# qradiolink/qradiolink

Measured on AMD Instinct MI355X. Metric: IQ MSamples/sec through RX demod chain, higher is better.
Workload: dtype f32

## Files before the change

include/qrl_hip.h:

```cpp
#ifndef QRL_HIP_H
#define QRL_HIP_H
#include <stddef.h>
#include <stdint.h>

#ifdef __cplusplus
extern "C" {
#endif

typedef enum {
    QRL_OK = 0,
    QRL_ERR_ARG = -1,
    QRL_ERR_NO_DEVICE = -2,
    QRL_ERR_HIP = -3,
    QRL_ERR_NOMEM = -4,
    QRL_ERR_TOO_BIG = -5,
    QRL_ERR_STATE = -6
} qrl_status;

enum {
    QRL_MODEM_BPSK2K = 0, QRL_MODEM_QPSK20K = 1, QRL_MODEM_QPSKVIDEO = 2, QRL_MODEM_4FSK2K = 3, QRL_MODEM_4FSK10KFM = 4, QRL_MODEM_4FSK2KFM = 5, QRL_MODEM_4FSK1KFM = 6, QRL_MODEM_QPSK2K = 7,
    QRL_MODEM_NBFM2500 = 8, QRL_MODEM_NBFM5000 = 9, QRL_MODEM_WBFM = 10, QRL_MODEM_USB2500 = 11, QRL_MODEM_LSB2500 = 12, QRL_MODEM_CW600USB = 13 , QRL_MODEM_AM5000 = 14,
    QRL_MODEM_2FSK2KFM = 15, QRL_MODEM_2FSK1KFM = 16, QRL_MODEM_2FSK2K = 17, QRL_MODEM_2FSK1K = 18,
    QRL_MODEM_2FSK10KFM = 19, QRL_MODEM_GMSK2K = 20, QRL_MODEM_GMSK1K = 21, QRL_MODEM_GMSK10K = 22,
    QRL_MODEM_BPSK1K = 24, QRL_MODEM_BPSK8 = 25 , QRL_MODEM_QPSK250K = 26, QRL_MODEM_4FSK100K = 27, QRL_MODEM_M17 = 40, QRL_MODEM_DMR = 41
// ... 8 lines not shown
const char* qrl_last_error(void);
const char* qrl_version(void);

typedef struct {
    int modem_type;
    int use_mode_defaults;
    int sps, samp_rate, carrier_freq, filter_width, fm;
    int device_samp_rate;
    double carrier_offset_hz;
    int batch;
    size_t max_chunk;
    void* hip_stream;
    int enable_side_outputs;
    int time_domain_samp_rate;
    double time_domain_filter_width;
} qrl_demod_config;

typedef struct {
    float* filtered;      size_t filtered_cap;
    float* constellation; size_t constellation_cap;
    uint8_t* bits_a;      size_t bits_cap;
    uint8_t* bits_b;
    uint32_t* counts;
    float* audio;         size_t audio_cap;
} qrl_demod_out;

int qrl_demod_create(qrl_ctx* ctx, const qrl_demod_config* cfg, qrl_demod** out);
void qrl_demod_destroy(qrl_demod* d);
int qrl_demod_reset(qrl_demod* d);
int qrl_demod_set_carrier_offset(qrl_demod* d, double carrier_offset_hz);
int qrl_demod_set_carrier_offsets(qrl_demod* d, const double* hz);
#define QRL_DMO_RECORD_BYTES 40
int qrl_demod_set_dmo_output(qrl_demod* d, uint8_t* frames, size_t cap_frames, uint32_t* counts);
enum { QRL_OPT_OVERLAP = 1, QRL_OPT_UNFUSED_DEC2 = 2, QRL_OPT_FLL_SLIM = 3 , QRL_OPT_GROUPED = 4, QRL_OPT_INPUT_RESIDENT = 5 };
int qrl_demod_set_option(qrl_demod* d, int option, int value);
int qrl_demod_out_caps(const qrl_demod* d, size_t n, size_t* filtered_cap, size_t* constellation_cap, size_t* bits_cap);
int qrl_demod_audio_cap(const qrl_demod* d, size_t n, size_t* audio_cap);
int qrl_demod_set_squelch(qrl_demod* d, double db);
int qrl_demod_time_domain_cap(const qrl_demod* d, size_t n, size_t* cap);
int qrl_demod_set_time_domain_output(qrl_demod* d, float* samples, size_t cap, uint32_t* counts);
int qrl_demod_set_ctcss(qrl_demod* d, float tone_hz);
int qrl_demod_set_agc(qrl_demod* d, float attack, float decay);
int qrl_demod_set_filter_width(qrl_demod* d, int filter_width);
int qrl_demod_set_gain(qrl_demod* d, float value);

int qrl_demod_process(qrl_demod* d, const float* iq, size_t stride, size_t n, const qrl_demod_out* out);
int qrl_demod_process_sc16(qrl_demod* d, const int16_t* iq, size_t stride, size_t n, const qrl_demod_out* out);
int qrl_demod_set_sc16_scale(qrl_demod* d, float scale);
int qrl_demod_sync(qrl_demod* d);
void* qrl_demod_stream(qrl_demod* d);
int qrl_demod_internal_streams(qrl_demod* d, void* out[3]);
int qrl_demod_stream_wait(qrl_demod* d, void* hip_stream);

int qrl_demod_profile(qrl_demod* d, int enable);
int qrl_demod_profile_read(qrl_demod* d, double* kernel_ms, uint64_t* launches, const char** kernel_name);

int qrl_demod_process_host(qrl_demod* d, const float* iq_host, size_t stride, size_t n,
                           uint8_t* bits_a_host, uint8_t* bits_b_host, size_t bits_cap, uint32_t* counts_host);
int qrl_demod_process_sc16_host(qrl_demod* d, const int16_t* iq_host, size_t stride, size_t n,
                                uint8_t* bits_a_host, uint8_t* bits_b_host, size_t bits_cap, uint32_t* counts_host);

typedef struct qrl_mod qrl_mod;
typedef struct {
    int modem_type;
    int use_mode_defaults;
    int sps, samp_rate, carrier_freq, filter_width, fm;
    int batch;
// ... 178 lines not shown
```

qradiolink_amd/__init__.py:

```python
import ctypes as C
import os

import numpy as np

_HERE = os.path.dirname(os.path.abspath(__file__))
LIB_PATH = os.environ.get("QRL_LIB_PATH") or os.path.join(_HERE, "libqrl_hip.so")

MODEM_2FSK2KFM, MODEM_2FSK1KFM, MODEM_2FSK2K, MODEM_2FSK1K, MODEM_2FSK10KFM = 15, 16, 17, 18, 19
MODEM_GMSK2K, MODEM_GMSK1K, MODEM_GMSK10K = 20, 21, 22
MODEM_QPSK250K = 26
MODEM_QPSK20K, MODEM_QPSKVIDEO, MODEM_QPSK2K = 1, 2, 7
MODEM_BPSK2K, MODEM_BPSK1K = 0, 24
MODEM_4FSK2K, MODEM_4FSK10KFM, MODEM_4FSK2KFM, MODEM_4FSK1KFM, MODEM_4FSK100K = 3, 4, 5, 6, 27
MODEM_BPSK8 = 25
MODEM_NBFM2500, MODEM_NBFM5000, MODEM_WBFM, MODEM_AM5000 = 8, 9, 10, 14
MODEM_USB2500, MODEM_LSB2500, MODEM_CW600USB = 11, 12, 13
MODEM_M17 = 40
MODEM_DMR = 41
OPT_OVERLAP, OPT_UNFUSED_DEC2, OPT_FLL_SLIM, OPT_GROUPED, OPT_INPUT_RESIDENT = 1, 2, 3, 4, 5
CHAN_OPT_LEGACY_PFB, CHAN_OPT_LEGACY_TAIL, CHAN_OPT_SERIAL_TAIL = 1, 2, 3
WIN_HAMMING, WIN_HANN, WIN_BLACKMAN, WIN_RECTANGULAR, WIN_BLACKMAN_HARRIS = 0, 1, 2, 3, 5


class QrlError(RuntimeError):
    pass


class _Config(C.Structure):
    _fields_ = [("modem_type", C.c_int), ("use_mode_defaults", C.c_int), ("sps", C.c_int), ("samp_rate", C.c_int),
                ("carrier_freq", C.c_int), ("filter_width", C.c_int), ("fm", C.c_int), ("device_samp_rate", C.c_int),
                ("carrier_offset_hz", C.c_double), ("batch", C.c_int), ("max_chunk", C.c_size_t),
                ("hip_stream", C.c_void_p), ("enable_side_outputs", C.c_int), ("time_domain_samp_rate", C.c_int), ("time_domain_filter_width", C.c_double)]


class _ModConfig(C.Structure):
    _fields_ = [("modem_type", C.c_int), ("use_mode_defaults", C.c_int), ("sps", C.c_int), ("samp_rate", C.c_int),
                ("carrier_freq", C.c_int), ("filter_width", C.c_int), ("fm", C.c_int), ("batch", C.c_int),
                ("max_bytes", C.c_size_t), ("hip_stream", C.c_void_p), ("bb_gain", C.c_float),
                ("device_samp_rate", C.c_int), ("carrier_offset_hz", C.c_double)]


class _ChanConfig(C.Structure):
    _fields_ = [("num_channels", C.c_int), ("channel_first", C.c_int), ("channel_count", C.c_int), ("batch", C.c_int),
                ("max_chunk", C.c_size_t), ("hip_stream", C.c_void_p), ("form", C.c_int), ("channel_separation", C.c_int),
                ("decimation", C.c_int), ("filter_width", C.c_int)]


class _SynthConfig(C.Structure):
    _fields_ = [("num_channels", C.c_int), ("filter_width", C.c_int), ("batch", C.c_int), ("max_samples", C.c_size_t),
                ("hip_stream", C.c_void_p), ("bb_gain", C.c_float), ("single_carrier", C.c_int)]


# ... 1029 lines not shown
```

qradiolink_amd/csrc/demod.hpp:

```cpp
#pragma once
#include "host_common.hpp"
#include "firdes.hpp"
#include <utility>

namespace qrl {

inline std::vector<float> decim_layout(const std::vector<float>& h, int D, int Jpad)
{
    std::vector<float> t((size_t)D * Jpad, 0.0f);
    for (size_t k = 0; k < h.size(); ++k) t[(k % D) * Jpad + k / D] = h[k];
    return t;
}
inline std::vector<float> resamp_layout(const std::vector<float>& h, int I, int Jp)
{
    std::vector<float> t((size_t)I * Jp, 0.0f);
    for (size_t k = 0; k < h.size(); ++k) t[(k % I) * Jp + k / I] = h[k];
    return t;
}
inline std::vector<float2> to_f2(const std::vector<std::complex<float>>& v)
{
    std::vector<float2> r(v.size());
    for (size_t i = 0; i < v.size(); ++i) r[i] = make_float2(v[i].real(), v[i].imag());
    return r;
}
// ... 63 lines not shown
    DevBuf<float> rs, filt, mf; int Jp = 0, nf = 0;
    DevBuf<float2> ra, rb, rc, rd, sym; uint32_t mask = 0, sym_mask = 0;
    DevBuf<DsssState> st; DevBuf<DsssTailState> tail;
    float a1 = 0, b1 = 0, a2 = 0, b2 = 0;
    uint64_t n5 = 0, nsy = 0;
    int build(qrl_demod& d, size_t max2);
    int init_state(qrl_demod& d);
    int stages(qrl_demod& d, uint64_t n2_0, uint64_t n2_1, const qrl_demod_out* out, uint32_t* counts);
};

}

using namespace qrl;

struct qrl_demod {
    qrl_ctx* ctx = nullptr;
    qrl_demod_config cfg{};
    hipStream_t stream = nullptr;
    bool own_stream = false;
    hipStream_t tail = nullptr;
    hipStream_t fecs = nullptr;
    hipEvent_t ev_q[2] = {nullptr, nullptr}, ev_fec[2] = {nullptr, nullptr}; bool q_valid[2] = {false, false};
    bool grouped = false, grouped_capable = false, fec_deferred = false; FecParams fec_pending{}; int fec_pending_slot = 0;
    DevBuf<uint64_t> qp_snap;
    hipEvent_t ev_ff = nullptr, ev_tail = nullptr;
    hipStream_t pre = nullptr; hipEvent_t ev_pre = nullptr, ev_fe[2] = {nullptr, nullptr}; bool fe_valid[2] = {false, false}; bool pre_pending = false;
    bool input_resident = false;
    hipEvent_t ev_user[4] = {nullptr, nullptr, nullptr, nullptr};
    bool tail_pending = false;
    bool qpsk_fll = false, fsk4_disc = false;
    bool m17 = false;
    DevBuf<float2> s2g, disc4_taps; DevBuf<float> sym4_taps; int disc4_nt = 0, sym4_nt = 0;
    bool fll_slim = false;
    bool d2f_capable = false, d2f = false; DevBuf<float> d2f_taps;
    bool overlap = false, overlap_capable = false; hipEvent_t ev_tail2[2] = {nullptr, nullptr}; bool tail2_valid[2] = {false, false}; uint64_t call_no = 0;
    enum Family { F_2FSK, F_GMSK, F_QPSK, F_DMR, F_4FSK, F_BPSK, F_DSSS, F_ANALOG } fam = F_2FSK;
    int branches = 2;

    int fe_decim = 1, interp = 1, decim = 1, target = 0, sps_eff = 0;
    bool fm = false;

    DecimStage fe;
    DecimStage first;
    DecimStage scope; DevBuf<float2> s_scope; uint32_t scope_mask = 0; uint64_t n_scope = 0; int scope_D = 10;
    float2* scope_out = nullptr; size_t scope_cap = 0; uint32_t* scope_counts = nullptr;
    DevBuf<float> rs_taps; int rs_Jp = 0;
    DevBuf<float> filt_taps; int filt_nt = 0;
    DevBuf<float> symf_taps; int symf_nt = 0;
    DevBuf<float2> disc_up, disc_lo; int disc_nt = 0;
    DevBuf<float> ff_tf, ff_ts; DevBuf<float2> ff_up, ff_lo;
    DevBuf<float2> fll_lo, fll_up; float fll_alpha = 0, fll_beta = 0, fll_maxf = 0;
    DevBuf<float> atan_tab, mmse_tab;
    float demod_gain = 0;
    float ss_alpha = 0, ss_beta = 0, ss_maxp = 0, ss_minp = 0;

    Rotator rot;

    DevBuf<float2> hist_a, hist_b; uint32_t hist_len = 0; bool hist_flip = false;
    DevBuf<float2> s1, s2, s2l, s2f; DevBuf<float> s2d, s3; DevBuf<uint8_t> soft;
    uint32_t s1_mask = 0, s2_mask = 0, soft_mask = 0;
    DevBuf<FllState> fll_st; DevBuf<SymSyncState> ss_st; DevBuf<FecState> fec_st;
    DevBuf<DmoState> dmo_st; DevBuf<uint32_t> dmo_golay; uint8_t* dmo_out = nullptr; uint32_t dmo_cap = 0; uint32_t* dmo_counts = nullptr;
    DevBuf<QpskState> qp_st; DevBuf<float> tanh_tab;
    float c1_alpha = 0, c1_beta = 0, c2_alpha = 0, c2_beta = 0; float2 qp_rot{};
    DevBuf<uint32_t> counts_scratch;
    AnalogChain an;
// ... 49 lines not shown
```

qradiolink_amd/csrc/engine.cpp:

```cpp
#include "demod.hpp"
#include <cmath>
#include <cstdlib>
#include <memory>
#include <new>

#ifndef QRL_FEC_GATE_US
#define QRL_FEC_GATE_US 30u
#endif
#ifndef QRL_DEV_SKIP
#define QRL_DEV_SKIP 0
#endif

int qrl_demod::flush_fec(bool behind_front_end)
{
    if (!fec_deferred) return QRL_OK;
    fec_deferred = false;
    HIPCHK(hipStreamWaitEvent(fecs, ev_q[fec_pending_slot], 0));
    if (behind_front_end) {
        HIPCHK(hipStreamWaitEvent(fecs, ev_ff, 0));
        launch_fec_gate(QRL_FEC_GATE_US, fecs);
    }
    launch_fec(fec_pending, cfg.batch, fecs);
    HIPCHK(hipEventRecord(ev_fec[fec_pending_slot], fecs));
    return QRL_OK;
// ... 359 lines not shown
    {
        HistParams h{};
        h.in = in; h.in_stride = stride; h.n0 = n_in0; h.n = (uint32_t)n;
        h.hist_old = hist_old; h.hist_new = hist_new; h.hist_len = hist_len;
        h.rot_enable = 1; rot.fill(h);
        h.in_fmt = fmt; h.in_scale = sc16_scale;
        if (pre) { HIPCHK(hipEventRecord(ev_fe[slot], stream)); fe_valid[slot] = true; }
        if (use_pre) {
            if (fe_valid[slot ^ 1]) HIPCHK(hipStreamWaitEvent(pre, ev_fe[slot ^ 1], 0));
            launch_hist_save(h, B, pre);
            HIPCHK(hipEventRecord(ev_pre, pre));
            pre_pending = true;
        } else launch_hist_save(h, B, stream);
        hist_flip = !hist_flip;
    }
    if (overlap) {
        HIPCHK(hipEventRecord(ev_ff, stream));
        HIPCHK(hipStreamWaitEvent(tail, ev_ff, 0));
        HIPCHK(hipMemsetAsync(counts, 0, (size_t)B * 4 * sizeof(uint32_t), tail));
    }
    const uint32_t c2 = (uint32_t)(n2_1 - n2_0);
    if (fam == F_DSSS || fam == F_ANALOG) {
        if (int rr = fam == F_DSSS ? ds.stages(*this, n2_0, n2_1, out, counts) : an.stages(*this, n2_0, n2_1, out, counts)) return rr;
        HIPCHK(hipGetLastError());
        if (take_launch_error()) return QRL_ERR_HIP;
        n_in = n_in1; n1 = n1_1; n2 = n2_1; ++call_no;
        return QRL_OK;
    }
    RingC filt_in = r2;
    if (fam == F_2FSK || fam == F_BPSK || (fam == F_QPSK && qpsk_fll)) {
        FllParams f{};
        f.in = r2; f.out = r2l; f.q0 = n2_0; f.count = c2; f.st = fll_st.p;
        f.lower = fll_lo.p; f.upper = fll_up.p; f.nt = fam == F_2FSK ? 16 : 32; f.alpha = fll_alpha; f.beta = fll_beta; f.max_freq = fll_maxf;
        f.slim = fll_slim ? 1 : 0;
        if (!(QRL_DEV_SKIP & 1)) launch_fll(f, B, cs);
        filt_in = r2l;
    }
    const bool fused_2fsk = fam == F_2FSK && !fm && filt_nt <= 41 && disc_nt <= 41 && symf_nt <= 25;
    if (fam == F_DMR) {
        RingC dem_in = r2;
        if (m17) {
            FirCcfParams f{};
            f.in = r2; f.out = r2f; f.q0 = n2_0; f.count = c2; f.taps = filt_taps.p; f.nt = filt_nt;
            f.port = fport.p; f.port_cap = fport.cap; f.counts = counts;
            launch_fir_ccf(f, B, cs);
            dem_in = r2f;
        }
        QuadDemodParams q{}; q.in = dem_in; q.out = r2d; q.q0 = n2_0; q.count = c2; q.gain = demod_gain; q.atan_tab = atan_tab.p;
        launch_quad_demod(q, B, cs);
        if (!overlap && tail_pending) { HIPCHK(hipStreamWaitEvent(stream, ev_tail, 0)); tail_pending = false; }
        FirFffParams f{}; f.in = r2d; f.out = r3; f.q0 = n2_0; f.count = c2; f.taps = symf_taps.p; f.nt = symf_nt;
        launch_fir_fff(f, B, cs);
        if (!overlap) { HIPCHK(hipEventRecord(ev_ff, stream)); HIPCHK(hipStreamWaitEvent(tail, ev_ff, 0)); }
    } else if (fused_2fsk) {
        if (!overlap && tail_pending) { HIPCHK(hipStreamWaitEvent(stream, ev_tail, 0)); tail_pending = false; }
        Fsk2FfParams f{};
        f.in = filt_in; f.out = r3; f.q0 = n2_0; f.count = c2;
        f.tf = ff_tf.p; f.nf = fsk2_ff_padded(filt_nt); f.up = ff_up.p; f.lo = ff_lo.p; f.nb = fsk2_ff_padded(disc_nt);
        f.ts = ff_ts.p; f.ns = fsk2_ff_padded(symf_nt);
        f.port = fport.p; f.port_cap = fport.cap; f.counts = counts;
        if (!(QRL_DEV_SKIP & 2)) launch_2fsk_ff(f, B, cs);
        if (!overlap) { HIPCHK(hipEventRecord(ev_ff, stream)); HIPCHK(hipStreamWaitEvent(tail, ev_ff, 0)); }
    } else {
        if (!d2f) {
            FirCcfParams f{};
            f.in = filt_in; f.out = r2f; f.q0 = n2_0; f.count = c2; f.taps = filt_taps.p; f.nt = filt_nt;
            f.port = fport.p; f.port_cap = fport.cap; f.counts = counts;
// ... 228 lines not shown
    HIPCHK(hipEventRecord(d->ev_user[3], d->pre ? d->pre : d->stream));
    for (auto e : d->ev_user) HIPCHK(hipStreamWaitEvent(user, e, 0));
    return QRL_OK;
}
int qrl_demod_set_dmo_output(qrl_demod* d, uint8_t* frames, size_t cap_frames, uint32_t* counts)
{
    if (!d) return QRL_ERR_ARG;
    if (d->fam != qrl_demod::F_DMR || d->m17) return qrl_set_error(QRL_ERR_ARG, "the DMO slicer sits behind port 3 of gr_demod_dmr: QRL_MODEM_DMR only");
    if (!frames) { if (int rs = d->sync_all()) return rs; d->dmo_out = nullptr; return QRL_OK; }
    if (!counts || cap_frames < 1 || cap_frames > 0xFFFFFFFFu) return QRL_ERR_ARG;
    int r;
    if (!d->dmo_st.p) {
        if (int rs = d->sync_all()) return rs;
        if ((r = d->dmo_st.alloc(d->cfg.batch)) || (r = d->dmo_golay.upload(golay1987_table()))) return r;
        if ((r = d->init_dmo_state())) return r;
    }
    d->dmo_out = frames; d->dmo_cap = (uint32_t)cap_frames; d->dmo_counts = counts;
    return QRL_OK;
}
int qrl_demod_set_option(qrl_demod* d, int option, int value)
{
    if (!d) return QRL_ERR_ARG;
    switch (option) {
    case QRL_OPT_OVERLAP:
        if (value != 0 && !d->overlap_capable) return qrl_set_error(QRL_ERR_ARG, "overlapped mode exists for the 2FSK family only");
        if (int rs = d->sync_all()) return rs;
        d->overlap = value != 0;
        d->tail2_valid[0] = d->tail2_valid[1] = false;
        return QRL_OK;
    case QRL_OPT_FLL_SLIM:
        if (int rs = d->sync_all()) return rs;
        d->fll_slim = value != 0;
        return QRL_OK;
    case QRL_OPT_GROUPED:
        if (value != 0 && !d->grouped_capable) return qrl_set_error(QRL_ERR_ARG, "the grouped order exists for the gr_demod_qpsk chain only");
        if (int rs = d->sync_all()) return rs;
        d->grouped = value != 0;
        return QRL_OK;
    case QRL_OPT_INPUT_RESIDENT: {
        if (int rs = d->sync_all()) return rs;
        if (value != 0 && d->pre) {
            DecimStage& st = d->fe.used ? d->fe : d->first;
            if (st.edge_len && !st.edge_b.p) if (int r = st.edge_b.alloc((size_t)d->cfg.batch * st.edge_len)) return qrl_set_error(r, "edge scratch");
        }
        d->input_resident = value != 0;
        return QRL_OK;
    }
    case QRL_OPT_UNFUSED_DEC2:
        if (!d->d2f_capable) return qrl_set_error(QRL_ERR_ARG, "this chain has no fused 1:2 decimator + shaping filter");
        if (d->n_in != 0) return qrl_set_error(QRL_ERR_STATE, "QRL_OPT_UNFUSED_DEC2 can only be set before the first sample (the two forms carry different state)");
        d->d2f = value == 0;
        return QRL_OK;
    default:
        return qrl_set_error(QRL_ERR_ARG, "unknown option");
    }
}
int qrl_demod_out_caps(const qrl_demod* d, size_t n, size_t* fcap, size_t* ccap, size_t* bcap)
{
    if (!d) return QRL_ERR_ARG;
    const CallCounts cc = d->call_counts(n);
    const size_t ns = cc.nsym;
    if (fcap) *fcap = cc.n2;
    if (ccap) *ccap = ns;
    if (bcap) *bcap = d->fam == qrl_demod::F_DMR ? 2 * ns + 8 : d->fam == qrl_demod::F_QPSK || d->fam == qrl_demod::F_4FSK ? (ns / 80 + 2) * 80 : (ns / 2 / 80 + 2) * 80;
    return QRL_OK;
}
// ... 141 lines not shown
```

qradiolink_amd/csrc/engine.hpp:

```cpp
#pragma once
#include <hip/hip_runtime.h>
#include <stdint.h>
#include <vector>
#include "zero_runs.hpp"
#include "decim_plan.hpp"

namespace qrl {

hipError_t dyn_lds_limit(const void* kernel, int bytes);
bool take_launch_error();

int create_role_stream(hipStream_t* s, int priority, const char* role);

struct RingC { float2* p; uint32_t mask; };
struct RingF { float* p; uint32_t mask; };
struct RingB { uint8_t* p; uint32_t mask; };

template <class Pp>
__device__ __forceinline__ void rot_select(Pp& c, const Pp& p, uint32_t b)
{
    c = p; c.rot_acc = p.rot_acc_s[b]; c.rot_inc = p.rot_inc_s[b]; c.rot_lo = p.rot_lo + (size_t)b * 512;
}
#define ROT_VIEW(T, PS, P, SRC, B) T P##_ps_; if constexpr (PS) rot_select(P##_ps_, SRC, (uint32_t)(B)); const T& P = (PS) ? P##_ps_ : SRC
std::vector<float2> rot_fine_table(uint64_t inc);
// ... 73 lines not shown
    RingC in_ring;
    RingC out;
    uint64_t q0; uint32_t q_count;
    const float* taps;
    int I, D, Jp;
    int rot_enable; uint64_t rot_acc; uint64_t rot_inc; uint64_t rot_nbase; const float2* rot_lo;
    float2* port; size_t port_cap; uint32_t* port_counts;
    const uint64_t* rot_acc_s; const uint64_t* rot_inc_s;
};
void launch_resamp(const ResampParams& p, int batch, hipStream_t s);

struct FirCcfParams { RingC in; RingC out; uint64_t q0; uint32_t count; const float* taps; int nt;
                      float2* port; size_t port_cap; uint32_t* counts; };
struct FirFffParams { RingF in; RingF out; uint64_t q0; uint32_t count; const float* taps; int nt; };
struct QuadDemodParams { RingC in; RingF out; uint64_t q0; uint32_t count; float gain; const float* atan_tab;
                         RingF out2; float gain2;
                         int16_t* s16; size_t s16_cap; float s16_level, s16_scale; uint32_t* s16_counts; };
struct Disc2fskParams { RingC in; RingF out; uint64_t q0; uint32_t count; const float2* up; const float2* lo; int nt; };
struct Disc4fskParams { RingC in; RingC out; uint64_t q0; uint32_t count; const float2* taps; int nt; };
void launch_disc_4fsk(const Disc4fskParams& p, int batch, hipStream_t s);
struct Fsk2FfParams { RingC in; RingF out; uint64_t q0; uint32_t count;
                      const float* tf; int nf; const float2* up; const float2* lo; int nb; const float* ts; int ns;
                      float2* port; size_t port_cap; uint32_t* counts; };
void launch_2fsk_ff(const Fsk2FfParams& p, int batch, hipStream_t s);
int fsk2_ff_padded(int n);
void launch_fir_ccf(const FirCcfParams& p, int batch, hipStream_t s);
void launch_fir_fff(const FirFffParams& p, int batch, hipStream_t s);
void launch_quad_demod(const QuadDemodParams& p, int batch, hipStream_t s);
void launch_disc_2fsk(const Disc2fskParams& p, int batch, hipStream_t s);

struct FllState { float phase, freq; float2 dl[32]; };
struct FllParams { RingC in; RingC out; uint64_t q0; uint32_t count; FllState* st;
                   const float2* lower; const float2* upper; int nt; float alpha, beta, max_freq;
                   int slim; };
void launch_fll(const FllParams& p, int batch, hipStream_t s);

struct SymSyncState { uint64_t ii; uint64_t oo; float mu, avg, inst; float x0, x1, x2, d0, d1, d2; };
struct SymSyncParams {
    RingF in; uint64_t avail;
    RingB soft;
    SymSyncState* st;
    const float* mmse;
    float alpha, beta, maxp, minp;
    int ted; float soft_mul, soft_add;
    int slicer;
    float tail_scale;
    int tail;
    uint8_t* bits; size_t bits_cap;
    float2* port; size_t port_cap; uint32_t* counts;
    int slim;
};
void launch_symsync_ff(const SymSyncParams& p, int batch, hipStream_t s);

struct QpskState {
    uint64_t ii, oo;
    float gain;
    float c1_phase, c1_freq;
    float mu, avg, inst;
    float2 x0, x1, x2, d0, d1, d2;
    float c2_phase, c2_freq;
    float2 dprev;
    float2 hist[16];
};
struct QpskParams {
    RingC in; uint64_t np0, avail;
    RingB soft; QpskState* st;
    const float* mmse; const float* tanh_tab;
// ... 203 lines not shown
```

qradiolink_amd/csrc/kernels_ff.hip:

```cpp
#include "devmath.hpp"
#include "engine.hpp"
#include <cstdlib>

namespace qrl {

__device__ __forceinline__ float2 ringc_at(const RingC& r, int b, int64_t i)
{
    if (i < 0) return make_float2(0.f, 0.f);
    return r.p[(size_t)b * (r.mask + 1u) + ((uint32_t)i & r.mask)];
}
__device__ __forceinline__ float ringf_at(const RingF& r, int b, int64_t i)
{
    if (i < 0) return 0.f;
    return r.p[(size_t)b * (r.mask + 1u) + ((uint32_t)i & r.mask)];
}

__global__ __launch_bounds__(256) void k_fir_ccf(const FirCcfParams P)
{
    const int b = blockIdx.y;
    const uint32_t t = blockIdx.x * 256u + threadIdx.x;
    if (t >= P.count) return;
    if (t == 0 && P.counts) P.counts[b * 4 + 0] = P.count;
    const int64_t n = (int64_t)(P.q0 + t);
    float ar = 0.f, ai = 0.f;
// ... 198 lines not shown
    ItemT cur[4], nxt[4];
#pragma unroll
    for (int s = 0; s < 4; ++s) cur[s] = tile[s * PITCH + w];
    auto quad = [&](int q) {
        --w;
#pragma unroll
        for (int s = 0; s < 4; ++s) nxt[s] = tile[s * PITCH + w];
        const TapT h0 = taps[4 * q], h1 = taps[4 * q + 1], h2 = taps[4 * q + 2], h3 = taps[4 * q + 3];
        fma4(h0, cur[0], cur[1], cur[2], cur[3]);
        fma4(h1, nxt[3], cur[0], cur[1], cur[2]);
        fma4(h2, nxt[2], nxt[3], cur[0], cur[1]);
        fma4(h3, nxt[1], nxt[2], nxt[3], cur[0]);
#pragma unroll
        for (int s = 0; s < 4; ++s) cur[s] = nxt[s];
    };
    if constexpr (NQ > 0) {
#pragma unroll 4
        for (int q = 0; q < NQ; ++q) quad(q);
    } else {
        for (int q = 0; q < nq_rt; ++q) quad(q);
    }
}

template <int NQF, int NQB, int NQS>
__global__ __launch_bounds__(256) void k_2fsk_ff(const Fsk2FfParams P)
{
    __shared__ float2 lt[4 * FF_PL];
    __shared__ float2 ft[4 * FF_PF];
    __shared__ float dt[4 * FF_PD];
    const int b = blockIdx.y, tid = threadIdx.x;
    const int hf = P.nf - 1, hb = P.nb - 1, hs = P.ns - 1;
    const int T = 1024 - hb - hs;
    const int64_t n0t = (int64_t)P.q0 + (int64_t)blockIdx.x * T;
    const int nl = 1024 + hf, nd = T + hs;
    if (tid < 4) { lt[tid * FF_PL] = make_float2(0.f, 0.f); ft[tid * FF_PF] = make_float2(0.f, 0.f); dt[tid * FF_PD] = 0.f; }
    {
        float2 v[5];
#pragma unroll
        for (int it = 0; it < 5; ++it) {
            const int64_t a = n0t - (hf + hb + hs) + tid + 256 * it;
            v[it] = P.in.p[(size_t)b * (P.in.mask + 1u) + ((uint32_t)a & P.in.mask)];
            if (a < 0) v[it] = make_float2(0.f, 0.f);
        }
#pragma unroll
        for (int it = 0; it < 5; ++it) {
            const int i = tid + 256 * it;
            if (i < nl) lt[(i & 3) * FF_PL + (i >> 2) + 1] = v[it];
        }
    }
    __syncthreads();
    {
        float2 a[4] = {{0.f, 0.f}, {0.f, 0.f}, {0.f, 0.f}, {0.f, 0.f}};
        ff_window4<FF_PL, NQF>(lt, tid + (hf >> 2) + 1, (hf >> 2) + 1, P.tf,
                          [&](float h, const float2& x0, const float2& x1, const float2& x2, const float2& x3) {
                              a[0].x = fmaf(h, x0.x, a[0].x); a[0].y = fmaf(h, x0.y, a[0].y);
                              a[1].x = fmaf(h, x1.x, a[1].x); a[1].y = fmaf(h, x1.y, a[1].y);
                              a[2].x = fmaf(h, x2.x, a[2].x); a[2].y = fmaf(h, x2.y, a[2].y);
                              a[3].x = fmaf(h, x3.x, a[3].x); a[3].y = fmaf(h, x3.y, a[3].y);
                          });
#pragma unroll
        for (int r = 0; r < 4; ++r) {
            const bool neg = n0t - (hb + hs) + 4 * tid + r < 0;
            ft[r * FF_PF + tid + 1] = neg ? make_float2(0.f, 0.f) : a[r];
        }
    }
    __syncthreads();
    if (4 * tid < nd) {
        float ar[4] = {0.f, 0.f, 0.f, 0.f}, ai[4] = {0.f, 0.f, 0.f, 0.f}, br[4] = {0.f, 0.f, 0.f, 0.f}, bi[4] = {0.f, 0.f, 0.f, 0.f};
        const int nq = NQB > 0 ? NQB : (hb >> 2) + 1;
        int w = tid + (hb >> 2) + 1;
        float2 cur[4], nxt[4];
#pragma unroll
        for (int s = 0; s < 4; ++s) cur[s] = ft[s * FF_PF + w];
        auto step = [&](const float2 h, const float2& x0, const float2& x1, const float2& x2, const float2& x3) {
            const float2 xs[4] = {x0, x1, x2, x3};
#pragma unroll
            for (int r = 0; r < 4; ++r) {
                ar[r] = fmaf(h.x, xs[r].x, ar[r]); ai[r] = fmaf(h.x, xs[r].y, ai[r]);
                br[r] = fmaf(h.y, xs[r].x, br[r]); bi[r] = fmaf(h.y, xs[r].y, bi[r]);
            }
        };
        auto quad = [&](int q) {
            --w;
#pragma unroll
            for (int s = 0; s < 4; ++s) nxt[s] = ft[s * FF_PF + w];
            step(P.up[4 * q], cur[0], cur[1], cur[2], cur[3]);
            step(P.up[4 * q + 1], nxt[3], cur[0], cur[1], cur[2]);
            step(P.up[4 * q + 2], nxt[2], nxt[3], cur[0], cur[1]);
            step(P.up[4 * q + 3], nxt[1], nxt[2], nxt[3], cur[0]);
#pragma unroll
            for (int s = 0; s < 4; ++s) cur[s] = nxt[s];
        };
        if constexpr (NQB > 0) {
#pragma unroll 4
            for (int q = 0; q < NQB; ++q) quad(q);
        } else {
            for (int q = 0; q < nq; ++q) quad(q);
        }
#pragma unroll
        for (int r = 0; r < 4; ++r) {
            const float ur = ar[r] - bi[r], ui = ai[r] + br[r], lr = ar[r] + bi[r], li = ai[r] - br[r];
            const float mu = sqrtf(ur * ur + ui * ui);
            const float ml = sqrtf(lr * lr + li * li);
            float v = mu / ml;
            if (!(v >= 0.0f)) v = 0.0f;
            if (v > 2.0f) v = 2.0f;
            dt[r * FF_PD + tid + 1] = (n0t - hs + 4 * tid + r < 0) ? 0.f : v + (-1.0f);
        }
    }
    __syncthreads();
    if (4 * tid < T) {
        float a[4] = {0.f, 0.f, 0.f, 0.f};
        ff_window4<FF_PD, NQS>(dt, tid + (hs >> 2) + 1, (hs >> 2) + 1, P.ts,
                          [&](float h, float x0, float x1, float x2, float x3) {
                              a[0] = fmaf(h, x0, a[0]); a[1] = fmaf(h, x1, a[1]); a[2] = fmaf(h, x2, a[2]); a[3] = fmaf(h, x3, a[3]);
                          });
        const uint32_t t0 = blockIdx.x * (uint32_t)T + 4u * tid;
        if (t0 == 0 && P.counts) P.counts[b * 4 + 0] = P.count;
        const int wf = tid + ((hb + hs) >> 2) + 1;
#pragma unroll
        for (int r = 0; r < 4; ++r) {
            const uint32_t t = t0 + r;
            if (t < P.count) {
                const int64_t n = n0t + 4 * tid + r;
                P.out.p[(size_t)b * (P.out.mask + 1u) + ((uint32_t)n & P.out.mask)] = a[r];
                if (P.port && t < P.port_cap) P.port[(size_t)b * P.port_cap + t] = ft[r * FF_PF + wf];
            }
        }
    }
}
int fsk2_ff_padded(int n) { return (n - 1 + 3) / 4 * 4 + 1; }
void launch_2fsk_ff(const Fsk2FfParams& p, int batch, hipStream_t s)
{
    if (!p.count) return;
    const int T = 1024 - (p.nb - 1) - (p.ns - 1);
    const dim3 grid((p.count + T - 1) / T, batch);
    static const bool rt = [] { const char* e = getenv("QRL_FF_RUNTIME_TAPS"); return e && atoi(e) != 0; }();
    const int qf = (p.nf - 1) / 4 + 1, qb = (p.nb - 1) / 4 + 1, qs = (p.ns - 1) / 4 + 1;
    if (!rt && qf == 11 && qb == 11 && qs == 7) hipLaunchKernelGGL((k_2fsk_ff<11, 11, 7>), grid, dim3(256), 0, s, p);
    else hipLaunchKernelGGL((k_2fsk_ff<0, 0, 0>), grid, dim3(256), 0, s, p);
}

}
```

qradiolink_amd/csrc/kernels_loops.hip:

```cpp
#include "devmath.hpp"
#include "engine.hpp"

namespace qrl {


#ifndef QRL_FLL_CH
#define QRL_FLL_CH 32
#endif
#ifndef QRL_FLL_TH
#define QRL_FLL_TH 256
#endif
template <int CTRL> __device__ __forceinline__ float dpp_quad(float v)
{
    return __builtin_bit_cast(float, __builtin_amdgcn_mov_dpp(__builtin_bit_cast(int, v), CTRL, 0xF, 0xF, true));
}

template <int NT, int FLL_TH, int FLL_CH>
__global__ __launch_bounds__(FLL_TH) void k_fll(const FllParams P, int batch)
{
    constexpr int FLL_NS = FLL_TH / 4;
    constexpr int GL = NT / 4;
    __shared__ float2 win[FLL_NS][FLL_CH + 1];
    __shared__ float2 tl[NT], tu[NT];
    __shared__ float2 dump[FLL_TH];
    const int tid = threadIdx.x;
    const int sl = tid >> 2, g = tid & 3;
    const int b0 = blockIdx.x * FLL_NS;
    const int b = b0 + sl;
    const bool active = b < batch;
    for (int k = tid; k < NT; k += FLL_TH) { tl[k] = P.lower[k]; tu[k] = P.upper[k]; }
    float phase = 0.f, freq = 0.f;
    float2 dl[GL];
    if (active) {
        const FllState& s = P.st[b];
        phase = s.phase; freq = s.freq;
#pragma unroll
        for (int t = 0; t < GL; ++t) dl[t] = s.dl[g * GL + t];
    } else {
#pragma unroll
        for (int t = 0; t < GL; ++t) dl[t] = make_float2(0.f, 0.f);
    }
    const int nstreams = min(FLL_NS, batch - b0);
    __syncthreads();
    float2 hu[GL], hl[GL];
#pragma unroll
    for (int t = 0; t < GL; ++t) { hu[t] = tu[g * GL + t]; hl[t] = tl[g * GL + t]; }
    constexpr int NPT = FLL_NS * FLL_CH / FLL_TH;
    float2 pre[NPT];
    auto preload = [&](uint32_t c0) {
#pragma unroll
        for (int i = 0; i < NPT; ++i) {
            const int idx = tid + FLL_TH * i, s = min(idx / FLL_CH, nstreams - 1), k = idx % FLL_CH;
            const int64_t a = (int64_t)(P.q0 + c0 + k) - NT;
            const float2 v = P.in.p[(size_t)(b0 + s) * (P.in.mask + 1u) + ((uint32_t)a & P.in.mask)];
            pre[i] = a >= 0 ? v : make_float2(0.f, 0.f);
        }
    };
    preload(0);
    for (uint32_t c0 = 0; c0 < P.count; c0 += FLL_CH) {
        const int len = min((uint32_t)FLL_CH, P.count - c0);
        __syncthreads();
#pragma unroll
        for (int i = 0; i < NPT; ++i) { const int idx = tid + FLL_TH * i; win[idx / FLL_CH][idx % FLL_CH] = pre[i]; }
        __syncthreads();
        if (c0 + FLL_CH < P.count) preload(c0 + FLL_CH);
        if (active) {
            for (int k = 0; k < len; ++k) {
                const float2 x = win[sl][k];
                const float2 nco = sincos_rad(phase);
                float2 carry;
                carry.x = dpp_quad<0x90>(dl[GL - 1].x);
                carry.y = dpp_quad<0x90>(dl[GL - 1].y);
#pragma unroll
                for (int t = GL - 1; t > 0; --t) dl[t] = dl[t - 1];
                float ur = 0.f, ui = 0.f, lr = 0.f, li = 0.f;
#pragma unroll
                for (int t = GL - 1; t >= 1; --t) {
                    const float2 v = dl[t];
                    ur = fmaf(hu[t].x, v.x, ur); ur = fmaf(-hu[t].y, v.y, ur);
                    ui = fmaf(hu[t].x, v.y, ui); ui = fmaf(hu[t].y, v.x, ui);
                    lr = fmaf(hl[t].x, v.x, lr); lr = fmaf(-hl[t].y, v.y, lr);
                    li = fmaf(hl[t].x, v.y, li); li = fmaf(hl[t].y, v.x, li);
                }
                const float2 y = cmul(x, nco);
                *(g == 0 ? &win[sl][k] : &dump[tid]) = y;
                dl[0] = g == 0 ? y : carry;
                {
                    const float2 v = dl[0];
                    ur = fmaf(hu[0].x, v.x, ur); ur = fmaf(-hu[0].y, v.y, ur);
                    ui = fmaf(hu[0].x, v.y, ui); ui = fmaf(hu[0].y, v.x, ui);
                    lr = fmaf(hl[0].x, v.x, lr); lr = fmaf(-hl[0].y, v.y, lr);
                    li = fmaf(hl[0].x, v.y, li); li = fmaf(hl[0].y, v.x, li);
                }
                ur = ur + dpp_quad<0xB1>(ur); ui = ui + dpp_quad<0xB1>(ui); lr = lr + dpp_quad<0xB1>(lr); li = li + dpp_quad<0xB1>(li);
                ur = ur + dpp_quad<0x4E>(ur); ui = ui + dpp_quad<0x4E>(ui); lr = lr + dpp_quad<0x4E>(lr); li = li + dpp_quad<0x4E>(li);
                const float error = (lr * lr + li * li) - (ur * ur + ui * ui);
                freq = freq + P.beta * error;
                phase = phase + freq + P.alpha * error;
                phase = phase_wrap(phase);
                freq = __builtin_fminf(__builtin_fmaxf(freq, -P.max_freq), P.max_freq);
            }
        }
        __syncthreads();
#pragma unroll
        for (int i = 0; i < NPT; ++i) {
            const int idx = tid + FLL_TH * i, s = idx / FLL_CH, k = idx % FLL_CH;
            if (s < nstreams && k < len) P.out.p[(size_t)(b0 + s) * (P.out.mask + 1u) + ((uint32_t)(P.q0 + c0 + k) & P.out.mask)] = win[s][k];
        }
    }
    if (active) {
        FllState& s = P.st[b];
        if (g == 0) { s.phase = phase; s.freq = freq; }
#pragma unroll
        for (int t = 0; t < GL; ++t) s.dl[g * GL + t] = dl[t];
    }
}

void launch_fll(const FllParams& p, int batch, hipStream_t s)
{
    if (!p.count) return;
    if (p.slim) {
        dim3 grid((batch + 15) / 16), block(64);
        if (p.nt == 16) hipLaunchKernelGGL((k_fll<16, 64, 16>), grid, block, 0, s, p, batch);
        else            hipLaunchKernelGGL((k_fll<32, 64, 16>), grid, block, 0, s, p, batch);
        return;
    }
    constexpr int TH = QRL_FLL_TH;
    dim3 grid((batch + TH / 4 - 1) / (TH / 4)), block(TH);
    if (p.nt == 16) hipLaunchKernelGGL((k_fll<16, TH, QRL_FLL_CH>), grid, block, 0, s, p, batch);
    else            hipLaunchKernelGGL((k_fll<32, TH, QRL_FLL_CH>), grid, block, 0, s, p, batch);
}

template <int NS, int W> struct SsGeo {
    static constexpr int BACK = 16;
    static constexpr int COLS = BACK + W + 8;
    static constexpr int PITCH = COLS + 1;
    static constexpr int OMAX = W == 192 ? 56 : (W + 5) * 2 / 7 + 1;
    static constexpr int OPITCH = OMAX + 1;
    static constexpr size_t lds_bytes() { return (size_t)(2 * NS * PITCH + 4 + 129 * 8 + 2 * NS * OPITCH) * sizeof(float) + 2 * 64 * sizeof(int) + (2 * 64 + 64 + 2) * sizeof(uint64_t); }
};

__device__ __forceinline__ uint64_t wave_min_u64(uint64_t v)
{
#pragma unroll
    for (int off = 32; off > 0; off >>= 1) {
        const uint64_t o = __shfl_xor((unsigned long long)v, off, 64);
        v = o < v ? o : v;
    }
    return v;
}

template <int SS_NS, int SS_W, bool VEC = false, int SS_TH = 256>
__global__ __launch_bounds__(SS_TH) void k_symsync_ff(const SymSyncParams P, int batch)
{
    using G = SsGeo<SS_NS, SS_W>;
    constexpr int SS_BACK = G::BACK, SS_COLS = G::COLS, SS_PITCH = G::PITCH, SS_OMAX = G::OMAX, SS_OPITCH = G::OPITCH;
    extern __shared__ __align__(16) unsigned char ss_smem[];
    float* win = reinterpret_cast<float*>(ss_smem);
    float* mm = win + 2 * SS_NS * SS_PITCH + 4;
    float* osym = mm + 129 * 8;
    int* ocnt = reinterpret_cast<int*>(osym + 2 * SS_NS * SS_OPITCH);
    uint64_t* obase = reinterpret_cast<uint64_t*>(ocnt + 2 * 64);
    uint64_t* oo0 = obase + 2 * 64;
// ... 233 lines not shown
```

Baseline: 535,000.

## Make FLL lanes-per-stream configurable and trim FF kernel tail work

Generalizes the FLL band-edge kernel so each stream can be handled by 1, 2 or 4 lanes, with a new option and compile-time defaults that pick the lane count. Fewer lanes per stream mean fewer cross-lane DPP reductions and more streams per block, at the cost of more serial FMAs per lane. The defaults stay at 4 lanes, so the default path matches the old layout apart from the refactor into a step lambda. Separately, the fused FF kernel now bounds its loads and compute loops by the valid sample count of the last block, which skips loads and filtering past the end of the data.

```diff
diff --git a/include/qrl_hip.h b/include/qrl_hip.h
--- a/include/qrl_hip.h
+++ b/include/qrl_hip.h
@@ -64,7 +64,8 @@
 int qrl_demod_set_carrier_offsets(qrl_demod* d, const double* hz);
 #define QRL_DMO_RECORD_BYTES 40
 int qrl_demod_set_dmo_output(qrl_demod* d, uint8_t* frames, size_t cap_frames, uint32_t* counts);
-enum { QRL_OPT_OVERLAP = 1, QRL_OPT_UNFUSED_DEC2 = 2, QRL_OPT_FLL_SLIM = 3 , QRL_OPT_GROUPED = 4, QRL_OPT_INPUT_RESIDENT = 5 };
+enum { QRL_OPT_OVERLAP = 1, QRL_OPT_UNFUSED_DEC2 = 2, QRL_OPT_FLL_SLIM = 3 , QRL_OPT_GROUPED = 4, QRL_OPT_INPUT_RESIDENT = 5,
+       QRL_OPT_FLL_LANES = 6  };
 int qrl_demod_set_option(qrl_demod* d, int option, int value);
 int qrl_demod_out_caps(const qrl_demod* d, size_t n, size_t* filtered_cap, size_t* constellation_cap, size_t* bits_cap);
 int qrl_demod_audio_cap(const qrl_demod* d, size_t n, size_t* audio_cap);
diff --git a/qradiolink_amd/__init__.py b/qradiolink_amd/__init__.py
--- a/qradiolink_amd/__init__.py
+++ b/qradiolink_amd/__init__.py
@@ -17,7 +17,7 @@
 MODEM_USB2500, MODEM_LSB2500, MODEM_CW600USB = 11, 12, 13
 MODEM_M17 = 40
 MODEM_DMR = 41
-OPT_OVERLAP, OPT_UNFUSED_DEC2, OPT_FLL_SLIM, OPT_GROUPED, OPT_INPUT_RESIDENT = 1, 2, 3, 4, 5
+OPT_OVERLAP, OPT_UNFUSED_DEC2, OPT_FLL_SLIM, OPT_GROUPED, OPT_INPUT_RESIDENT, OPT_FLL_LANES = 1, 2, 3, 4, 5, 6
 CHAN_OPT_LEGACY_PFB, CHAN_OPT_LEGACY_TAIL, CHAN_OPT_SERIAL_TAIL = 1, 2, 3
 WIN_HAMMING, WIN_HANN, WIN_BLACKMAN, WIN_RECTANGULAR, WIN_BLACKMAN_HARRIS = 0, 1, 2, 3, 5
 
diff --git a/qradiolink_amd/csrc/demod.hpp b/qradiolink_amd/csrc/demod.hpp
--- a/qradiolink_amd/csrc/demod.hpp
+++ b/qradiolink_amd/csrc/demod.hpp
@@ -119,6 +119,7 @@
     bool m17 = false;
     DevBuf<float2> s2g, disc4_taps; DevBuf<float> sym4_taps; int disc4_nt = 0, sym4_nt = 0;
     bool fll_slim = false;
+    int fll_lanes = 0;
     bool d2f_capable = false, d2f = false; DevBuf<float> d2f_taps;
     bool overlap = false, overlap_capable = false; hipEvent_t ev_tail2[2] = {nullptr, nullptr}; bool tail2_valid[2] = {false, false}; uint64_t call_no = 0;
     enum Family { F_2FSK, F_GMSK, F_QPSK, F_DMR, F_4FSK, F_BPSK, F_DSSS, F_ANALOG } fam = F_2FSK;
diff --git a/qradiolink_amd/csrc/engine.cpp b/qradiolink_amd/csrc/engine.cpp
--- a/qradiolink_amd/csrc/engine.cpp
+++ b/qradiolink_amd/csrc/engine.cpp
@@ -415,7 +415,7 @@
         FllParams f{};
         f.in = r2; f.out = r2l; f.q0 = n2_0; f.count = c2; f.st = fll_st.p;
         f.lower = fll_lo.p; f.upper = fll_up.p; f.nt = fam == F_2FSK ? 16 : 32; f.alpha = fll_alpha; f.beta = fll_beta; f.max_freq = fll_maxf;
-        f.slim = fll_slim ? 1 : 0;
+        f.slim = fll_slim ? 1 : 0; f.lanes = fll_lanes;
         if (!(QRL_DEV_SKIP & 1)) launch_fll(f, B, cs);
         filt_in = r2l;
     }
@@ -710,6 +710,11 @@
         if (int rs = d->sync_all()) return rs;
         d->fll_slim = value != 0;
         return QRL_OK;
+    case QRL_OPT_FLL_LANES:
+        if (value != 1 && value != 2 && value != 4) return qrl_set_error(QRL_ERR_ARG, "QRL_OPT_FLL_LANES takes 1, 2 or 4");
+        if (int rs = d->sync_all()) return rs;
+        d->fll_lanes = value;
+        return QRL_OK;
     case QRL_OPT_GROUPED:
         if (value != 0 && !d->grouped_capable) return qrl_set_error(QRL_ERR_ARG, "the grouped order exists for the gr_demod_qpsk chain only");
         if (int rs = d->sync_all()) return rs;
diff --git a/qradiolink_amd/csrc/engine.hpp b/qradiolink_amd/csrc/engine.hpp
--- a/qradiolink_amd/csrc/engine.hpp
+++ b/qradiolink_amd/csrc/engine.hpp
@@ -129,7 +129,8 @@
 struct FllState { float phase, freq; float2 dl[32]; };
 struct FllParams { RingC in; RingC out; uint64_t q0; uint32_t count; FllState* st;
                    const float2* lower; const float2* upper; int nt; float alpha, beta, max_freq;
-                   int slim; };
+                   int slim;
+                   int lanes; };
 void launch_fll(const FllParams& p, int batch, hipStream_t s);
 
 struct SymSyncState { uint64_t ii; uint64_t oo; float mu, avg, inst; float x0, x1, x2, d0, d1, d2; };
diff --git a/qradiolink_amd/csrc/kernels_ff.hip b/qradiolink_amd/csrc/kernels_ff.hip
--- a/qradiolink_amd/csrc/kernels_ff.hip
+++ b/qradiolink_amd/csrc/kernels_ff.hip
@@ -254,24 +254,25 @@
     const int hf = P.nf - 1, hb = P.nb - 1, hs = P.ns - 1;
     const int T = 1024 - hb - hs;
     const int64_t n0t = (int64_t)P.q0 + (int64_t)blockIdx.x * T;
-    const int nl = 1024 + hf, nd = T + hs;
+    const int nv = (int)min((uint32_t)T, P.count - blockIdx.x * (uint32_t)T);
+    const int n1 = nv + hb + hs, n2 = nv + hs;
     if (tid < 4) { lt[tid * FF_PL] = make_float2(0.f, 0.f); ft[tid * FF_PF] = make_float2(0.f, 0.f); dt[tid * FF_PD] = 0.f; }
     {
         float2 v[5];
 #pragma unroll
         for (int it = 0; it < 5; ++it) {
             const int64_t a = n0t - (hf + hb + hs) + tid + 256 * it;
-            v[it] = P.in.p[(size_t)b * (P.in.mask + 1u) + ((uint32_t)a & P.in.mask)];
-            if (a < 0) v[it] = make_float2(0.f, 0.f);
+            v[it] = make_float2(0.f, 0.f);
+            if (tid + 256 * it < n1 + hf && a >= 0) v[it] = P.in.p[(size_t)b * (P.in.mask + 1u) + ((uint32_t)a & P.in.mask)];
         }
 #pragma unroll
         for (int it = 0; it < 5; ++it) {
             const int i = tid + 256 * it;
-            if (i < nl) lt[(i & 3) * FF_PL + (i >> 2) + 1] = v[it];
-        }
-    }
-    __syncthreads();
-    {
+            if (i < n1 + hf) lt[(i & 3) * FF_PL + (i >> 2) + 1] = v[it];
+        }
+    }
+    __syncthreads();
+    if (4 * tid < n1) {
         float2 a[4] = {{0.f, 0.f}, {0.f, 0.f}, {0.f, 0.f}, {0.f, 0.f}};
         ff_window4<FF_PL, NQF>(lt, tid + (hf >> 2) + 1, (hf >> 2) + 1, P.tf,
                           [&](float h, const float2& x0, const float2& x1, const float2& x2, const float2& x3) {
@@ -287,7 +288,7 @@
         }
     }
     __syncthreads();
-    if (4 * tid < nd) {
+    if (4 * tid < n2) {
         float ar[4] = {0.f, 0.f, 0.f, 0.f}, ai[4] = {0.f, 0.f, 0.f, 0.f}, br[4] = {0.f, 0.f, 0.f, 0.f}, bi[4] = {0.f, 0.f, 0.f, 0.f};
         const int nq = NQB > 0 ? NQB : (hb >> 2) + 1;
         int w = tid + (hb >> 2) + 1;
@@ -331,7 +332,7 @@
         }
     }
     __syncthreads();
-    if (4 * tid < T) {
+    if (4 * tid < nv) {
         float a[4] = {0.f, 0.f, 0.f, 0.f};
         ff_window4<FF_PD, NQS>(dt, tid + (hs >> 2) + 1, (hs >> 2) + 1, P.ts,
                           [&](float h, float x0, float x1, float x2, float x3) {
diff --git a/qradiolink_amd/csrc/kernels_loops.hip b/qradiolink_amd/csrc/kernels_loops.hip
--- a/qradiolink_amd/csrc/kernels_loops.hip
+++ b/qradiolink_amd/csrc/kernels_loops.hip
@@ -15,36 +15,39 @@
     return __builtin_bit_cast(float, __builtin_amdgcn_mov_dpp(__builtin_bit_cast(int, v), CTRL, 0xF, 0xF, true));
 }
 
-template <int NT, int FLL_TH, int FLL_CH>
+template <int NT, int FLL_TH, int FLL_CH, int LPS = 4>
 __global__ __launch_bounds__(FLL_TH) void k_fll(const FllParams P, int batch)
 {
-    constexpr int FLL_NS = FLL_TH / 4;
+    static_assert(LPS == 1 || LPS == 2 || LPS == 4, "lanes per stream");
+    constexpr int FLL_NS = FLL_TH / LPS;
     constexpr int GL = NT / 4;
+    constexpr int CPL = 4 / LPS;
+    constexpr int ML = CPL * GL;
     __shared__ float2 win[FLL_NS][FLL_CH + 1];
     __shared__ float2 tl[NT], tu[NT];
-    __shared__ float2 dump[FLL_TH];
+    __shared__ float2 dump[LPS == 4 ? FLL_TH : LPS == 2 ? FLL_NS : 1];
     const int tid = threadIdx.x;
-    const int sl = tid >> 2, g = tid & 3;
+    const int sl = tid / LPS, g = tid % LPS;
     const int b0 = blockIdx.x * FLL_NS;
     const int b = b0 + sl;
     const bool active = b < batch;
     for (int k = tid; k < NT; k += FLL_TH) { tl[k] = P.lower[k]; tu[k] = P.upper[k]; }
     float phase = 0.f, freq = 0.f;
-    float2 dl[GL];
+    float2 dl[ML];
     if (active) {
         const FllState& s = P.st[b];
         phase = s.phase; freq = s.freq;
 #pragma unroll
-        for (int t = 0; t < GL; ++t) dl[t] = s.dl[g * GL + t];
+        for (int t = 0; t < ML; ++t) dl[t] = s.dl[g * ML + t];
     } else {
 #pragma unroll
-        for (int t = 0; t < GL; ++t) dl[t] = make_float2(0.f, 0.f);
+        for (int t = 0; t < ML; ++t) dl[t] = make_float2(0.f, 0.f);
     }
     const int nstreams = min(FLL_NS, batch - b0);
     __syncthreads();
-    float2 hu[GL], hl[GL];
-#pragma unroll
-    for (int t = 0; t < GL; ++t) { hu[t] = tu[g * GL + t]; hl[t] = tl[g * GL + t]; }
+    float2 hu[ML], hl[ML];
+#pragma unroll
+    for (int t = 0; t < ML; ++t) { hu[t] = tu[g * ML + t]; hl[t] = tl[g * ML + t]; }
     constexpr int NPT = FLL_NS * FLL_CH / FLL_TH;
     float2 pre[NPT];
     auto preload = [&](uint32_t c0) {
@@ -56,6 +59,57 @@
             pre[i] = a >= 0 ? v : make_float2(0.f, 0.f);
         }
     };
+    auto step = [&](int k) __attribute__((always_inline)) {
+        const float2 x = win[sl][k];
+        const float2 nco = sincos_rad(phase);
+        float2 carry = make_float2(0.f, 0.f);
+        if constexpr (LPS == 4) { carry.x = dpp_quad<0x90>(dl[ML - 1].x); carry.y = dpp_quad<0x90>(dl[ML - 1].y); }
+        if constexpr (LPS == 2) { carry.x = dpp_quad<0xA0>(dl[ML - 1].x); carry.y = dpp_quad<0xA0>(dl[ML - 1].y); }
+#pragma unroll
+        for (int t = ML - 1; t > 0; --t) dl[t] = dl[t - 1];
+        float ur[CPL], ui[CPL], lr[CPL], li[CPL];
+#pragma unroll
+        for (int c = CPL - 1; c >= 0; --c) {
+            ur[c] = 0.f; ui[c] = 0.f; lr[c] = 0.f; li[c] = 0.f;
+#pragma unroll
+            for (int t = c * GL + GL - 1; t >= c * GL + (c == 0 ? 1 : 0); --t) {
+                const float2 v = dl[t];
+                ur[c] = fmaf(hu[t].x, v.x, ur[c]); ur[c] = fmaf(-hu[t].y, v.y, ur[c]);
+                ui[c] = fmaf(hu[t].x, v.y, ui[c]); ui[c] = fmaf(hu[t].y, v.x, ui[c]);
+                lr[c] = fmaf(hl[t].x, v.x, lr[c]); lr[c] = fmaf(-hl[t].y, v.y, lr[c]);
+                li[c] = fmaf(hl[t].x, v.y, li[c]); li[c] = fmaf(hl[t].y, v.x, li[c]);
+            }
+        }
+        const float2 y = cmul(x, nco);
+        if constexpr (LPS == 4) *(g == 0 ? &win[sl][k] : &dump[tid]) = y;
+        if constexpr (LPS == 2) *(g == 0 ? &win[sl][k] : &dump[sl]) = y;
+        if constexpr (LPS == 1) win[sl][k] = y;
+        if constexpr (LPS == 1) dl[0] = y; else dl[0] = g == 0 ? y : carry;
+        {
+            const float2 v = dl[0];
+            ur[0] = fmaf(hu[0].x, v.x, ur[0]); ur[0] = fmaf(-hu[0].y, v.y, ur[0]);
+            ui[0] = fmaf(hu[0].x, v.y, ui[0]); ui[0] = fmaf(hu[0].y, v.x, ui[0]);
+            lr[0] = fmaf(hl[0].x, v.x, lr[0]); lr[0] = fmaf(-hl[0].y, v.y, lr[0]);
+            li[0] = fmaf(hl[0].x, v.y, li[0]); li[0] = fmaf(hl[0].y, v.x, li[0]);
+        }
+        float sur, sui, slr, sli;
+        if constexpr (LPS == 1) {
+            sur = (ur[0] + ur[1]) + (ur[2] + ur[3]); sui = (ui[0] + ui[1]) + (ui[2] + ui[3]);
+            slr = (lr[0] + lr[1]) + (lr[2] + lr[3]); sli = (li[0] + li[1]) + (li[2] + li[3]);
+        } else if constexpr (LPS == 2) {
+            sur = ur[0] + ur[1]; sui = ui[0] + ui[1]; slr = lr[0] + lr[1]; sli = li[0] + li[1];
+            sur = sur + dpp_quad<0xB1>(sur); sui = sui + dpp_quad<0xB1>(sui); slr = slr + dpp_quad<0xB1>(slr); sli = sli + dpp_quad<0xB1>(sli);
+        } else {
+            sur = ur[0]; sui = ui[0]; slr = lr[0]; sli = li[0];
+            sur = sur + dpp_quad<0xB1>(sur); sui = sui + dpp_quad<0xB1>(sui); slr = slr + dpp_quad<0xB1>(slr); sli = sli + dpp_quad<0xB1>(sli);
+            sur = sur + dpp_quad<0x4E>(sur); sui = sui + dpp_quad<0x4E>(sui); slr = slr + dpp_quad<0x4E>(slr); sli = sli + dpp_quad<0x4E>(sli);
+        }
+        const float error = (slr * slr + sli * sli) - (sur * sur + sui * sui);
+        freq = freq + P.beta * error;
+        phase = phase + freq + P.alpha * error;
+        phase = phase_wrap(phase);
+        freq = __builtin_fminf(__builtin_fmaxf(freq, -P.max_freq), P.max_freq);
+    };
     preload(0);
     for (uint32_t c0 = 0; c0 < P.count; c0 += FLL_CH) {
         const int len = min((uint32_t)FLL_CH, P.count - c0);
@@ -65,41 +119,7 @@
         __syncthreads();
         if (c0 + FLL_CH < P.count) preload(c0 + FLL_CH);
         if (active) {
-            for (int k = 0; k < len; ++k) {
-                const float2 x = win[sl][k];
-                const float2 nco = sincos_rad(phase);
-                float2 carry;
-                carry.x = dpp_quad<0x90>(dl[GL - 1].x);
-                carry.y = dpp_quad<0x90>(dl[GL - 1].y);
-#pragma unroll
-                for (int t = GL - 1; t > 0; --t) dl[t] = dl[t - 1];
-                float ur = 0.f, ui = 0.f, lr = 0.f, li = 0.f;
-#pragma unroll
-                for (int t = GL - 1; t >= 1; --t) {
-                    const float2 v = dl[t];
-                    ur = fmaf(hu[t].x, v.x, ur); ur = fmaf(-hu[t].y, v.y, ur);
-                    ui = fmaf(hu[t].x, v.y, ui); ui = fmaf(hu[t].y, v.x, ui);
-                    lr = fmaf(hl[t].x, v.x, lr); lr = fmaf(-hl[t].y, v.y, lr);
-                    li = fmaf(hl[t].x, v.y, li); li = fmaf(hl[t].y, v.x, li);
-                }
-                const float2 y = cmul(x, nco);
-                *(g == 0 ? &win[sl][k] : &dump[tid]) = y;
-                dl[0] = g == 0 ? y : carry;
-                {
-                    const float2 v = dl[0];
-                    ur = fmaf(hu[0].x, v.x, ur); ur = fmaf(-hu[0].y, v.y, ur);
-                    ui = fmaf(hu[0].x, v.y, ui); ui = fmaf(hu[0].y, v.x, ui);
-                    lr = fmaf(hl[0].x, v.x, lr); lr = fmaf(-hl[0].y, v.y, lr);
-                    li = fmaf(hl[0].x, v.y, li); li = fmaf(hl[0].y, v.x, li);
-                }
-                ur = ur + dpp_quad<0xB1>(ur); ui = ui + dpp_quad<0xB1>(ui); lr = lr + dpp_quad<0xB1>(lr); li = li + dpp_quad<0xB1>(li);
-                ur = ur + dpp_quad<0x4E>(ur); ui = ui + dpp_quad<0x4E>(ui); lr = lr + dpp_quad<0x4E>(lr); li = li + dpp_quad<0x4E>(li);
-                const float error = (lr * lr + li * li) - (ur * ur + ui * ui);
-                freq = freq + P.beta * error;
-                phase = phase + freq + P.alpha * error;
-                phase = phase_wrap(phase);
-                freq = __builtin_fminf(__builtin_fmaxf(freq, -P.max_freq), P.max_freq);
-            }
+            for (int k = 0; k < len; ++k) step(k);
         }
         __syncthreads();
 #pragma unroll
@@ -112,10 +132,25 @@
         FllState& s = P.st[b];
         if (g == 0) { s.phase = phase; s.freq = freq; }
 #pragma unroll
-        for (int t = 0; t < GL; ++t) s.dl[g * GL + t] = dl[t];
-    }
-}
-
+        for (int t = 0; t < ML; ++t) s.dl[g * ML + t] = dl[t];
+    }
+}
+
+#ifndef QRL_FLL_LANES_NT16
+#define QRL_FLL_LANES_NT16 4
+#endif
+#ifndef QRL_FLL_LANES_NT32
+#define QRL_FLL_LANES_NT32 4
+#endif
+#ifndef QRL_FLL_TH2
+#define QRL_FLL_TH2 128
+#endif
+template <int TH, int LPS> static void launch_fll_form(const FllParams& p, int batch, hipStream_t s)
+{
+    dim3 grid((batch + TH / LPS - 1) / (TH / LPS)), block(TH);
+    if (p.nt == 16) hipLaunchKernelGGL((k_fll<16, TH, QRL_FLL_CH, LPS>), grid, block, 0, s, p, batch);
+    else            hipLaunchKernelGGL((k_fll<32, TH, QRL_FLL_CH, LPS>), grid, block, 0, s, p, batch);
+}
 void launch_fll(const FllParams& p, int batch, hipStream_t s)
 {
     if (!p.count) return;
@@ -125,10 +160,10 @@
         else            hipLaunchKernelGGL((k_fll<32, 64, 16>), grid, block, 0, s, p, batch);
         return;
     }
-    constexpr int TH = QRL_FLL_TH;
-    dim3 grid((batch + TH / 4 - 1) / (TH / 4)), block(TH);
-    if (p.nt == 16) hipLaunchKernelGGL((k_fll<16, TH, QRL_FLL_CH>), grid, block, 0, s, p, batch);
-    else            hipLaunchKernelGGL((k_fll<32, TH, QRL_FLL_CH>), grid, block, 0, s, p, batch);
+    const int lanes = p.lanes ? p.lanes : p.nt == 16 ? QRL_FLL_LANES_NT16 : QRL_FLL_LANES_NT32;
+    if (lanes == 1)      launch_fll_form<64, 1>(p, batch, s);
+    else if (lanes == 2) launch_fll_form<QRL_FLL_TH2, 2>(p, batch, s);
+    else                 launch_fll_form<QRL_FLL_TH, 4>(p, batch, s);
 }
 
 template <int NS, int W> struct SsGeo {
```

Result: no change. 537,200, median of 6 (+0.4%).
